# JADGardner/neusky

Hardware: AMD Instinct MI355X
Metric: train rays/sec on NeRF-OSR lk2 @1024 rays x 96 samples (higher is better)
Workload: dtype f32 in memory; forward products: fp16 hi + residual split, 3 x v_mfma_f32_32x32x16_f16 per product on power-of-two pre-scaled operands, one fp32 accumulator (~2^-22): FiLM-SIREN chains and the SDF / albedo field alike; backward products: the same fp16 split on per-row / per-matrix pre-scaled gradien; 1 GPU; full NeuSky train step (BASELINE configs[2]): 1024 rays/GPU x 96 samples, proposal 256+96, 512 illumination directions (256 upper-hemisphere DDF queries/ray), illumination decoder = this project's FiLM-SIREN H = 128 (RENI-shaped: latent 100x3; the reference's configured Attention decoder is absent from its tree), hash L16 F2 T2^19 x2, 256-wide MLPs; fwd + losses + bwd + all-reduce + 5 Adam groups; rays_per_gpu=1024, samples_per_ray=96, illumination_directions=512, parallelism=ray-sharded dp1, launcher=self-spawned, launch=HIP graph replay (1 graph/step + all-reduce + 5 Adam launches)

## Files before the change

neusky_amd/csrc/wgrad_native.hip:

```cpp
#include "common.h"
#include "../../include/neusky_hip.h"

namespace {

typedef _Float16 f16x8 __attribute__((ext_vector_type(8)));
typedef float f32x16 __attribute__((ext_vector_type(16)));
typedef float f32x4 __attribute__((ext_vector_type(4)));
typedef short s16x4 __attribute__((__vector_size__(4 * sizeof(short))));
typedef __attribute__((address_space(3))) s16x4 lds_s16x4;

struct WgradProblem {
  const float* A;
  const float* B;
  float* dW;
  float* db;
  const float* a_scale_max;
  float b_scale;
  const float* b_scale_max;
  int nnt_a, nnt_b, ldw;
  int tile0;
  int lda, ldb;
  int wa, wb;
  int bias_rows;
  int bias_mod;
};
struct WgradArgs {
  WgradProblem p[NSKY_WGRAD_MAX_PROBLEMS];
  int n_problems, rows, row_blocks, blocks_per_split, n_tiles;
};

__device__ __forceinline__ float pow2_scale(float m, float& inv) {
  if (!(m > 0.0f) || !(m < 3.0e38f)) { inv = 1.0f; return 1.0f; }
  int e;
  (void)frexpf(m, &e);
  e = max(-100, min(100, e));
  inv = ldexpf(1.0f, e - 15);
  return ldexpf(1.0f, 15 - e);
}

__device__ __forceinline__ int xcd_contiguous(int id, int total) {
  const int xcd = id & 7, idx = id >> 3, per = total >> 3, rem = total & 7;
  return xcd * per + min(xcd, rem) + idx;
}

template <bool BF>
__device__ __forceinline__ f32x16 mma(f16x8 x, f16x8 y, f32x16 acc) {
  typedef __bf16 b16x8 __attribute__((ext_vector_type(8)));
  if (BF) return __builtin_amdgcn_mfma_f32_32x32x16_bf16(__builtin_bit_cast(b16x8, x), __builtin_bit_cast(b16x8, y), acc, 0, 0, 0);
  return __builtin_amdgcn_mfma_f32_32x32x16_f16(x, y, acc, 0, 0, 0);
}

template <int WM, int WN, int TM, int TN, bool RM>
__global__ __launch_bounds__(64 * WM * WN, WM * WN == 8 ? 1 : 2) void wgrad_native_kernel(WgradArgs a) {
  constexpr int NW = WM * WN;
  constexpr int NT = NW;
  static_assert(WM * TM == NT && WN * TN == NT, "square output block");
  constexpr int OPB = NT * 4096;
  constexpr int STAGE = 2 * OPB;
  extern __shared__ __attribute__((aligned(16))) unsigned char smem[];

  const int tid = threadIdx.x, lane = tid & 63, wave = tid >> 6;
  const int wm = wave / WN, wn = wave % WN;
  const int logical = xcd_contiguous(blockIdx.x, gridDim.x);
  const int gtile = logical % a.n_tiles, split = logical / a.n_tiles;
  int pi = 0;
  while (pi + 1 < a.n_problems && gtile >= a.p[pi + 1].tile0) ++pi;
  const WgradProblem& P = a.p[pi];
  const int tile = gtile - P.tile0;
  const int kblocks = P.nnt_b / NT;
  const int nb = tile / kblocks, kb = tile % kblocks;
  const int r_beg = split * a.blocks_per_split;
  const int r_end = min(a.row_blocks, r_beg + a.blocks_per_split);
  if (r_beg >= r_end) return;

  float a_inv = 1.0f;
  const float a_scale = P.a_scale_max ? pow2_scale(*P.a_scale_max, a_inv) : 1.0f;
  float b_unused;
  const float b_scale = P.b_scale_max ? pow2_scale(*P.b_scale_max, b_unused) : P.b_scale;
  const bool clamp_b = P.b_scale_max == nullptr;

  const int c = lane & 31, hh = lane >> 5;
  const int rq = lane >> 3, fq = lane & 7;
  const int fa = (nb * NT + wave) * 32 + 4 * fq, fb = (kb * NT + wave) * 32 + 4 * fq;
  const bool fa_ok = fa < P.wa, fb_ok = fb < P.wb;
  const float* pa = RM ? P.A + (long)r_beg * 32 * P.lda + min(fa, max(P.wa - 4, 0))
                       : P.A + ((long)r_beg * P.nnt_a + nb * NT + wave) * 1024 + lane * 4;
  const float* pb = RM ? P.B + (long)r_beg * 32 * P.ldb + min(fb, max(P.wb - 4, 0))
                       : P.B + ((long)r_beg * P.nnt_b + kb * NT + wave) * 1024 + lane * 4;
  const long a_step = RM ? 32l * P.lda : (long)P.nnt_a * 1024, b_step = RM ? 32l * P.ldb : (long)P.nnt_b * 1024;
  int rm_row0 = 0;
  f32x4 raw[8];
  const float* pa2 = pa;
  const float* pb2 = pb;
  auto reload = [&](int uu) {
    if (RM) {
      const int row = min(rm_row0 + 8 * (uu >> 1) + rq, a.rows - 1) - rm_row0;
      raw[uu] = __builtin_nontemporal_load(reinterpret_cast<const f32x4*>(((uu & 1) ? pb2 + (long)row * P.ldb : pa2 + (long)row * P.lda)));
    } else {
      raw[uu] = __builtin_nontemporal_load(reinterpret_cast<const f32x4*>(((uu & 1) ? pb2 : pa2) + (uu >> 1) * 256));
    }
  };
  float bias[4][4];
#pragma unroll
  for (int u = 0; u < 4; ++u)
#pragma unroll
    for (int i = 0; i < 4; ++i) bias[u][i] = 0.0f;
  const bool want_bias = P.db != nullptr && kb == 0;
  const int w_base = wave * 4096 + c * 64 + 8 * hh;
  const int w_swz = (c >> 1) & 3;
  typedef _Float16 f16x4 __attribute__((ext_vector_type(4)));
  typedef __bf16 b16x4 __attribute__((ext_vector_type(4)));
  auto stage_unit = [&](int uu, int row0, bool row_block_live, unsigned char* stage) {
    const int op = uu & 1, u = uu >> 1;
    const float s = op == 0 ? a_scale : b_scale;
    const int row = row0 + (RM ? 8 * u + rq : c);
    const bool live = row_block_live && row < a.rows && (!RM || (op == 0 ? fa_ok : fb_ok));
    const bool bias_on = op == 0 && row < P.bias_rows && (P.bias_mod <= 1 || (row % P.bias_mod) == 0);
    float v[4];
#pragma unroll
    for (int i = 0; i < 4; ++i) {
      v[i] = live ? raw[uu][i] * s : 0.0f;
      if (op == 1 && clamp_b) v[i] = __builtin_amdgcn_fmed3f(v[i], -65504.0f, 65504.0f);
      if (op == 0) bias[u][i] += bias_on ? v[i] : 0.0f;
    }
    unsigned char* img;
    if (RM) {
      const int r = 8 * u + rq;
      img = stage + op * OPB + wave * 4096 + r * 64 + 16 * ((fq >> 1) ^ ((r >> 1) & 3)) + 8 * (fq & 1);
      b16x4 h4, l4;
#pragma unroll
      for (int i = 0; i < 4; ++i) { h4[i] = (__bf16)v[i]; l4[i] = (__bf16)(v[i] - (float)h4[i]); }
      *reinterpret_cast<b16x4*>(img) = h4;
      *reinterpret_cast<b16x4*>(img + 2048) = l4;
    } else {
      img = stage + op * OPB + w_base + 16 * (u ^ w_swz);
      f16x4 h4, l4;
#pragma unroll
      for (int i = 0; i < 4; ++i) { h4[i] = (_Float16)v[i]; l4[i] = (_Float16)(v[i] - (float)h4[i]); }
      *reinterpret_cast<f16x4*>(img) = h4;
      *reinterpret_cast<f16x4*>(img + 2048) = l4;
    }
  };

  const int i16 = lane & 15, q = i16 >> 2, p = i16 & 3, gsel = (lane >> 4) & 1, h = lane >> 5;
  int t_off[2];
#pragma unroll
  for (int rd = 0; rd < 2; ++rd) {
    const int row = 8 * h + 4 * rd + q;
    t_off[rd] = row * 64 + 16 * ((2 * gsel + (p >> 1)) ^ ((row >> 1) & 3)) + 8 * (p & 1);
  }
  auto frag = [&](const unsigned char* img, int ks) -> f16x8 {
    const s16x4 lo4 = __builtin_amdgcn_ds_read_tr16_b64_v4i16((lds_s16x4*)(img + ks * 1024 + t_off[0]));
    const s16x4 hi4 = __builtin_amdgcn_ds_read_tr16_b64_v4i16((lds_s16x4*)(img + ks * 1024 + t_off[1]));
    typedef short s16x8 __attribute__((ext_vector_type(8)));
    const s16x8 v = {lo4[0], lo4[1], lo4[2], lo4[3], hi4[0], hi4[1], hi4[2], hi4[3]};
    return __builtin_bit_cast(f16x8, v);
  };

  f32x16 acc[TM][TN];
#pragma unroll
  for (int i = 0; i < TM; ++i)
#pragma unroll
    for (int j = 0; j < TN; ++j)
#pragma unroll
      for (int r = 0; r < 16; ++r) acc[i][j][r] = 0.0f;

  rm_row0 = r_beg * 32;
#pragma unroll
  for (int uu = 0; uu < 8; ++uu) reload(uu);
  {
    if (r_beg + 1 < r_end) { pa2 += a_step; pb2 += b_step; rm_row0 += 32; }
#pragma unroll
    for (int uu = 0; uu < 8; ++uu) {
      stage_unit(uu, r_beg * 32, true, smem);
      reload(uu);
    }
    if (r_beg + 2 < r_end) { pa2 += a_step; pb2 += b_step; rm_row0 += 32; }
  }
  static_assert(TN == 4 || TN == 2, "one staging unit per (k-step, X tile) point, or two");
  constexpr int UPP = 8 / (2 * TN);
  int cur = 0;
  for (int r = r_beg; r < r_end; ++r) {
    __syncthreads();
    const bool live = r + 1 < r_end;
    const unsigned char* st = smem + cur * STAGE;
    unsigned char* nxt = smem + (cur ^ 1) * STAGE;
#pragma unroll
    for (int ks = 0; ks < 2; ++ks) {
      f16x8 ah[TM], al[TM], bh[2], bl[2];
#pragma unroll
      for (int i = 0; i < TM; ++i) {
        ah[i] = frag(st + (wm * TM + i) * 4096, ks);
        al[i] = frag(st + (wm * TM + i) * 4096 + 2048, ks);
      }
      bh[0] = frag(st + OPB + (wn * TN) * 4096, ks);
      bl[0] = frag(st + OPB + (wn * TN) * 4096 + 2048, ks);
#pragma unroll
      for (int j = 0; j < TN; ++j) {
        if (j + 1 < TN) {
          bh[(j + 1) & 1] = frag(st + OPB + (wn * TN + j + 1) * 4096, ks);
          bl[(j + 1) & 1] = frag(st + OPB + (wn * TN + j + 1) * 4096 + 2048, ks);
        }
#pragma unroll
        for (int i = 0; i < TM; ++i) acc[i][j] = mma<RM>(al[i], bh[j & 1], acc[i][j]);
#pragma unroll
        for (int i = 0; i < TM; ++i) acc[i][j] = mma<RM>(ah[i], bl[j & 1], acc[i][j]);
#pragma unroll
        for (int i = 0; i < TM; ++i) acc[i][j] = mma<RM>(ah[i], bh[j & 1], acc[i][j]);
#pragma unroll
        for (int k = 0; k < UPP; ++k) {
          const int uu = (ks * TN + j) * UPP + k;
          stage_unit(uu, (r + 1) * 32, live, nxt);
          reload(uu);
        }
        __builtin_amdgcn_sched_barrier(0);
      }
    }
    if (r + 3 < r_end) { pa2 += a_step; pb2 += b_step; rm_row0 += 32; }
    cur ^= 1;
  }

  const float out_scale = a_inv / b_scale;
  const int n0 = (nb * NT + wm * TM) * 32, k0 = (kb * NT + wn * TN) * 32;
#pragma unroll
  for (int i = 0; i < TM; ++i)
#pragma unroll
    for (int j = 0; j < TN; ++j) {
      float* out = P.dW + (long)(n0 + 32 * i + 4 * h) * P.ldw + k0 + 32 * j + (lane & 31);
      const bool col_ok = k0 + 32 * j + (lane & 31) < P.wb;
#pragma unroll
      for (int g = 0; g < 16; ++g)
        if (col_ok && n0 + 32 * i + 4 * h + 8 * (g >> 2) + (g & 3) < P.wa)
          atomicAdd(out + (long)(8 * (g >> 2) + (g & 3)) * P.ldw, acc[i][j][g] * out_scale);
      __builtin_amdgcn_sched_barrier(0);
    }
  if (want_bias && RM) {
#pragma unroll
    for (int i = 0; i < 4; ++i) {
      float v = (bias[0][i] + bias[1][i]) + (bias[2][i] + bias[3][i]);
#pragma unroll
      for (int off = 8; off < 64; off <<= 1) v += __shfl_xor(v, off, 64);
      if (rq == 0 && fa + i < P.wa) atomicAdd(P.db + fa + i, v * a_inv);
    }
  } else if (want_bias) {
#pragma unroll
    for (int u = 0; u < 4; ++u)
#pragma unroll
      for (int i = 0; i < 4; ++i) {
        float v = bias[u][i];
#pragma unroll
        for (int off = 16; off > 0; off >>= 1) v += __shfl_xor(v, off, 64);
        if (c == 0 && (nb * NT + wave) * 32 + 8 * u + 4 * hh + i < P.wa) atomicAdd(P.db + (nb * NT + wave) * 32 + 8 * u + 4 * hh + i, v * a_inv);
      }
  }
}

}

extern "C" int nsky_wgrad_native_batch(const nsky_wgrad_problem* problems, int32_t n_problems, int32_t rows, nsky_stream_t stream) {
  NSKY_CHECK_ARG(problems && n_problems >= 1 && n_problems <= NSKY_WGRAD_MAX_PROBLEMS && rows >= 0,
                 "nsky_wgrad_native_batch: 1..%d problems expected, got %d", NSKY_WGRAD_MAX_PROBLEMS, n_problems);
  if (rows == 0) return NSKY_OK;
  WgradArgs a;
  const bool rm = problems[0].lda > 0;
  bool wide = true;
  for (int i = 0; i < n_problems; ++i) {
    const nsky_wgrad_problem& q = problems[i];
    NSKY_CHECK_ARG(q.dZ && q.X && q.dW, "nsky_wgrad_native_batch: problem %d: null argument", i);
    NSKY_CHECK_ARG((q.lda > 0) == rm && (q.ldb > 0) == rm, "nsky_wgrad_native_batch: problem %d: row-major and tile-native operands in one launch", i);
    if (rm) {
      NSKY_CHECK_ARG(q.width_a >= 4 && q.width_b >= 4 && q.width_a % 4 == 0 && q.width_b % 4 == 0 && q.lda >= q.width_a && q.ldb >= q.width_b &&
                         q.lda % 4 == 0 && q.ldb % 4 == 0, "nsky_wgrad_native_batch: problem %d: row-major widths / leading dimensions must be multiples of 4", i);
      NSKY_CHECK_ARG(q.ldw >= q.width_b && q.a_scale_max == nullptr, "nsky_wgrad_native_batch: problem %d: ldw %d < %d, or a scale with row-major operands", i,
                     q.ldw, q.width_b);
      wide = wide && q.width_a > 128 && q.width_b > 128;
    } else {
      NSKY_CHECK_ARG(q.nnt_a > 0 && q.nnt_b > 0 && q.nnt_a % 4 == 0 && q.nnt_b % 4 == 0,
                     "nsky_wgrad_native_batch: problem %d: both operands need a multiple of 128 features (got %d and %d tiles of 32)", i,
                     q.nnt_a, q.nnt_b);
      NSKY_CHECK_ARG(q.width_a >= 0 && q.width_a <= 32 * q.nnt_a && q.width_b >= 0 && q.width_b <= 32 * q.nnt_b,
                     "nsky_wgrad_native_batch: problem %d: widths %d / %d exceed the tiles", i, q.width_a, q.width_b);
      NSKY_CHECK_ARG(q.ldw >= (q.width_b > 0 ? q.width_b : 32 * q.nnt_b), "nsky_wgrad_native_batch: problem %d: ldw %d too small", i, q.ldw);
      int e = 0;
      NSKY_CHECK_ARG(q.b_scale > 0.0f && frexpf(q.b_scale, &e) == 0.5f, "nsky_wgrad_native_batch: problem %d: b_scale must be a power of two", i);
      wide = wide && q.nnt_a % 8 == 0 && q.nnt_b % 8 == 0;
    }
  }
  const int NT = wide ? 8 : 4;
  int tiles = 0;
  for (int i = 0; i < n_problems; ++i) {
    const nsky_wgrad_problem& q = problems[i];
    WgradProblem& P = a.p[i];
    P.A = q.dZ; P.B = q.X; P.dW = q.dW; P.db = q.db; P.a_scale_max = q.a_scale_max; P.b_scale = rm ? 1.0f : q.b_scale;
    P.b_scale_max = rm ? nullptr : q.b_scale_max;
    P.nnt_a = rm ? ceil_div(q.width_a, 32 * NT) * NT : q.nnt_a;
    P.nnt_b = rm ? ceil_div(q.width_b, 32 * NT) * NT : q.nnt_b;
    P.ldw = q.ldw; P.tile0 = tiles;
    P.lda = q.lda; P.ldb = q.ldb;
    P.wa = (rm || q.width_a > 0) ? q.width_a : 32 * q.nnt_a;
    P.wb = (rm || q.width_b > 0) ? q.width_b : 32 * q.nnt_b;
    P.bias_rows = q.bias_rows > 0 ? q.bias_rows : rows;
    P.bias_mod = rm ? 0 : q.bias_row_mod;
    tiles += (P.nnt_a / NT) * (P.nnt_b / NT);
  }
  a.n_problems = n_problems; a.rows = rows; a.n_tiles = tiles;
  a.row_blocks = ceil_div(rows, 32);
  const int slots = wide ? 256 : 512;
  int splits = slots / a.n_tiles;
  if (splits < 1) splits = 1;
  if (splits > a.row_blocks) splits = a.row_blocks;
  a.blocks_per_split = ceil_div(a.row_blocks, splits);
  splits = ceil_div(a.row_blocks, a.blocks_per_split);
  const dim3 grid(a.n_tiles * splits);
  const size_t smem = 2 * 2 * NT * 4096;
  static bool attr_set = [] {
    (void)hipFuncSetAttribute(reinterpret_cast<const void*>(&wgrad_native_kernel<4, 2, 2, 4, false>), hipFuncAttributeMaxDynamicSharedMemorySize, 160 * 1024);
    (void)hipFuncSetAttribute(reinterpret_cast<const void*>(&wgrad_native_kernel<2, 2, 2, 2, false>), hipFuncAttributeMaxDynamicSharedMemorySize, 160 * 1024);
    (void)hipFuncSetAttribute(reinterpret_cast<const void*>(&wgrad_native_kernel<4, 2, 2, 4, true>), hipFuncAttributeMaxDynamicSharedMemorySize, 160 * 1024);
    (void)hipFuncSetAttribute(reinterpret_cast<const void*>(&wgrad_native_kernel<2, 2, 2, 2, true>), hipFuncAttributeMaxDynamicSharedMemorySize, 160 * 1024);
    return true;
  }();
  (void)attr_set;
  const hipStream_t st = (hipStream_t)stream;
  if (wide && rm) hipLaunchKernelGGL((wgrad_native_kernel<4, 2, 2, 4, true>), grid, dim3(512), smem, st, a);
  else if (wide) hipLaunchKernelGGL((wgrad_native_kernel<4, 2, 2, 4, false>), grid, dim3(512), smem, st, a);
  else if (rm) hipLaunchKernelGGL((wgrad_native_kernel<2, 2, 2, 2, true>), grid, dim3(256), smem, st, a);
  else hipLaunchKernelGGL((wgrad_native_kernel<2, 2, 2, 2, false>), grid, dim3(256), smem, st, a);
  NSKY_CHECK_LAUNCH("nsky_wgrad_native_batch");
  return NSKY_OK;
}

extern "C" int nsky_wgrad_native(const float* dZ, int32_t nnt_a, const float* X, int32_t nnt_b, int32_t rows, float* dW, int32_t ldw,
                                 float* db, const float* a_scale_max, float b_scale, nsky_stream_t stream) {
  nsky_wgrad_problem q = {};
  q.dZ = dZ; q.nnt_a = nnt_a; q.X = X; q.nnt_b = nnt_b; q.dW = dW; q.ldw = ldw; q.db = db; q.a_scale_max = a_scale_max; q.b_scale = b_scale;
  return nsky_wgrad_native_batch(&q, 1, rows, stream);
}
```

Before: 51650 rays/s.

## Software-pipeline LDS fragment reads across k-steps in weight-gradient kernel

Restructures the wgrad MFMA main loop so the A/B fragments for the next k-step (including the first k-step of the next row block) are read from LDS while the current MFMAs run, with a barrier per k-step in place of one per row block. It also remaps per-lane global load offsets to 32-bit byte offsets from a wave-uniform base, makes the wave index scalar, shrinks the bias accumulators and replaces the modulo bias-row test with a power-of-two mask and an FMA. The aim is to hide LDS latency and cut address and VGPR cost, in exchange for an extra barrier per k-step and more intricate staging/swizzle indexing.

```diff
diff --git a/neusky_amd/csrc/wgrad_native.hip b/neusky_amd/csrc/wgrad_native.hip
--- a/neusky_amd/csrc/wgrad_native.hip
+++ b/neusky_amd/csrc/wgrad_native.hip
@@ -23,6 +23,7 @@
   int wa, wb;
   int bias_rows;
   int bias_mod;
+  int bias_mask;
 };
 struct WgradArgs {
   WgradProblem p[NSKY_WGRAD_MAX_PROBLEMS];
@@ -59,7 +60,7 @@
   constexpr int STAGE = 2 * OPB;
   extern __shared__ __attribute__((aligned(16))) unsigned char smem[];
 
-  const int tid = threadIdx.x, lane = tid & 63, wave = tid >> 6;
+  const int tid = threadIdx.x, lane = tid & 63, wave = __builtin_amdgcn_readfirstlane(tid >> 6);
   const int wm = wave / WN, wn = wave % WN;
   const int logical = xcd_contiguous(blockIdx.x, gridDim.x);
   const int gtile = logical % a.n_tiles, split = logical / a.n_tiles;
@@ -79,30 +80,31 @@
   const float b_scale = P.b_scale_max ? pow2_scale(*P.b_scale_max, b_unused) : P.b_scale;
   const bool clamp_b = P.b_scale_max == nullptr;
 
-  const int c = lane & 31, hh = lane >> 5;
+  const int c = lane & 15, hh = (lane >> 4) & 1, us = lane >> 5;
   const int rq = lane >> 3, fq = lane & 7;
   const int fa = (nb * NT + wave) * 32 + 4 * fq, fb = (kb * NT + wave) * 32 + 4 * fq;
   const bool fa_ok = fa < P.wa, fb_ok = fb < P.wb;
-  const float* pa = RM ? P.A + (long)r_beg * 32 * P.lda + min(fa, max(P.wa - 4, 0))
-                       : P.A + ((long)r_beg * P.nnt_a + nb * NT + wave) * 1024 + lane * 4;
-  const float* pb = RM ? P.B + (long)r_beg * 32 * P.ldb + min(fb, max(P.wb - 4, 0))
-                       : P.B + ((long)r_beg * P.nnt_b + kb * NT + wave) * 1024 + lane * 4;
+  const float* pa2 = RM ? P.A + (long)r_beg * 32 * P.lda : P.A + ((long)r_beg * P.nnt_a + nb * NT + wave) * 1024;
+  const float* pb2 = RM ? P.B + (long)r_beg * 32 * P.ldb : P.B + ((long)r_beg * P.nnt_b + kb * NT + wave) * 1024;
   const long a_step = RM ? 32l * P.lda : (long)P.nnt_a * 1024, b_step = RM ? 32l * P.ldb : (long)P.nnt_b * 1024;
+  const unsigned lane_off = 4u * (us * 256 + hh * 128 + c * 4);
+  const unsigned fa_off = 4u * min(fa, max(P.wa - 4, 0)), fb_off = 4u * min(fb, max(P.wb - 4, 0));
   int rm_row0 = 0;
   f32x4 raw[8];
-  const float* pa2 = pa;
-  const float* pb2 = pb;
   auto reload = [&](int uu) {
+    const char* base = reinterpret_cast<const char*>((uu & 1) ? pb2 : pa2);
+    unsigned off;
     if (RM) {
-      const int row = min(rm_row0 + 8 * (uu >> 1) + rq, a.rows - 1) - rm_row0;
-      raw[uu] = __builtin_nontemporal_load(reinterpret_cast<const f32x4*>(((uu & 1) ? pb2 + (long)row * P.ldb : pa2 + (long)row * P.lda)));
+      const unsigned row = min(rm_row0 + 8 * (uu >> 1) + rq, a.rows - 1) - rm_row0;
+      off = (uu & 1) ? row * 4u * P.ldb + fb_off : row * 4u * P.lda + fa_off;
     } else {
-      raw[uu] = __builtin_nontemporal_load(reinterpret_cast<const f32x4*>(((uu & 1) ? pb2 : pa2) + (uu >> 1) * 256));
-    }
+      off = lane_off + 4u * (((uu >> 1) & 1) * 512 + (uu >> 2) * 64);
+    }
+    raw[uu] = __builtin_nontemporal_load(reinterpret_cast<const f32x4*>(base + off));
   };
-  float bias[4][4];
-#pragma unroll
-  for (int u = 0; u < 4; ++u)
+  float bias[2][4];
+#pragma unroll
+  for (int u = 0; u < 2; ++u)
 #pragma unroll
     for (int i = 0; i < 4; ++i) bias[u][i] = 0.0f;
   const bool want_bias = P.db != nullptr && kb == 0;
@@ -113,15 +115,18 @@
   auto stage_unit = [&](int uu, int row0, bool row_block_live, unsigned char* stage) {
     const int op = uu & 1, u = uu >> 1;
     const float s = op == 0 ? a_scale : b_scale;
-    const int row = row0 + (RM ? 8 * u + rq : c);
+    const int row = row0 + (RM ? 8 * u + rq : 16 * (u >> 1) + c);
     const bool live = row_block_live && row < a.rows && (!RM || (op == 0 ? fa_ok : fb_ok));
-    const bool bias_on = op == 0 && row < P.bias_rows && (P.bias_mod <= 1 || (row % P.bias_mod) == 0);
+    bool row_in = P.bias_mask >= 0 ? (row & P.bias_mask) == 0 : true;
+    if (P.bias_mask < 0 && P.bias_mod > 1) row_in = (row % P.bias_mod) == 0;
+    const bool bias_on = op == 0 && (row < P.bias_rows) & row_in;
+    const float bias_w = bias_on ? 1.0f : 0.0f;
     float v[4];
 #pragma unroll
     for (int i = 0; i < 4; ++i) {
       v[i] = live ? raw[uu][i] * s : 0.0f;
       if (op == 1 && clamp_b) v[i] = __builtin_amdgcn_fmed3f(v[i], -65504.0f, 65504.0f);
-      if (op == 0) bias[u][i] += bias_on ? v[i] : 0.0f;
+      if (op == 0) bias[RM ? 0 : u & 1][i] = __builtin_fmaf(v[i], bias_w, bias[RM ? 0 : u & 1][i]);
     }
     unsigned char* img;
     if (RM) {
@@ -133,7 +138,7 @@
       *reinterpret_cast<b16x4*>(img) = h4;
       *reinterpret_cast<b16x4*>(img + 2048) = l4;
     } else {
-      img = stage + op * OPB + w_base + 16 * (u ^ w_swz);
+      img = stage + op * OPB + w_base + (u >> 1) * 1024 + 16 * ((2 * (u & 1) + us) ^ w_swz);
       f16x4 h4, l4;
 #pragma unroll
       for (int i = 0; i < 4; ++i) { h4[i] = (_Float16)v[i]; l4[i] = (_Float16)(v[i] - (float)h4[i]); }
@@ -177,29 +182,39 @@
     }
     if (r_beg + 2 < r_end) { pa2 += a_step; pb2 += b_step; rm_row0 += 32; }
   }
-  static_assert(TN == 4 || TN == 2, "one staging unit per (k-step, X tile) point, or two");
-  constexpr int UPP = 8 / (2 * TN);
+  static_assert(TN == 4 || TN == 2, "one staging unit per X tile and slot, or two");
+  constexpr int UPP = 4 / TN;
+  __syncthreads();
+  f16x8 ah[TM], al[TM], bh[2], bl[2];
+#pragma unroll
+  for (int i = 0; i < TM; ++i) {
+    ah[i] = frag(smem + (wm * TM + i) * 4096, 0);
+    al[i] = frag(smem + (wm * TM + i) * 4096 + 2048, 0);
+  }
+  bh[0] = frag(smem + OPB + (wn * TN) * 4096, 0);
+  bl[0] = frag(smem + OPB + (wn * TN) * 4096 + 2048, 0);
   int cur = 0;
   for (int r = r_beg; r < r_end; ++r) {
-    __syncthreads();
     const bool live = r + 1 < r_end;
     const unsigned char* st = smem + cur * STAGE;
     unsigned char* nxt = smem + (cur ^ 1) * STAGE;
 #pragma unroll
     for (int ks = 0; ks < 2; ++ks) {
-      f16x8 ah[TM], al[TM], bh[2], bl[2];
-#pragma unroll
-      for (int i = 0; i < TM; ++i) {
-        ah[i] = frag(st + (wm * TM + i) * 4096, ks);
-        al[i] = frag(st + (wm * TM + i) * 4096 + 2048, ks);
-      }
-      bh[0] = frag(st + OPB + (wn * TN) * 4096, ks);
-      bl[0] = frag(st + OPB + (wn * TN) * 4096 + 2048, ks);
+      const unsigned char* sn = ks == 0 ? st : nxt;
+      const int kn = ks ^ 1;
+      f16x8 nh[TM], nl[TM];
 #pragma unroll
       for (int j = 0; j < TN; ++j) {
-        if (j + 1 < TN) {
-          bh[(j + 1) & 1] = frag(st + OPB + (wn * TN + j + 1) * 4096, ks);
-          bl[(j + 1) & 1] = frag(st + OPB + (wn * TN + j + 1) * 4096 + 2048, ks);
+        const unsigned char* bn = j + 1 < TN ? st + OPB + (wn * TN + j + 1) * 4096 : sn + OPB + (wn * TN) * 4096;
+        const int kb_ = j + 1 < TN ? ks : kn;
+        bh[(j + 1) & 1] = frag(bn, kb_);
+        bl[(j + 1) & 1] = frag(bn + 2048, kb_);
+        if (j == 0) {
+#pragma unroll
+          for (int i = 0; i < TM; ++i) {
+            nh[i] = frag(sn + (wm * TM + i) * 4096, kn);
+            nl[i] = frag(sn + (wm * TM + i) * 4096 + 2048, kn);
+          }
         }
 #pragma unroll
         for (int i = 0; i < TM; ++i) acc[i][j] = mma<RM>(al[i], bh[j & 1], acc[i][j]);
@@ -209,12 +224,15 @@
         for (int i = 0; i < TM; ++i) acc[i][j] = mma<RM>(ah[i], bh[j & 1], acc[i][j]);
 #pragma unroll
         for (int k = 0; k < UPP; ++k) {
-          const int uu = (ks * TN + j) * UPP + k;
+          const int uu = ks * 4 + j * UPP + k;
           stage_unit(uu, (r + 1) * 32, live, nxt);
           reload(uu);
         }
         __builtin_amdgcn_sched_barrier(0);
       }
+      __syncthreads();
+#pragma unroll
+      for (int i = 0; i < TM; ++i) { ah[i] = nh[i]; al[i] = nl[i]; }
     }
     if (r + 3 < r_end) { pa2 += a_step; pb2 += b_step; rm_row0 += 32; }
     cur ^= 1;
@@ -237,20 +255,21 @@
   if (want_bias && RM) {
 #pragma unroll
     for (int i = 0; i < 4; ++i) {
-      float v = (bias[0][i] + bias[1][i]) + (bias[2][i] + bias[3][i]);
+      float v = bias[0][i];
 #pragma unroll
       for (int off = 8; off < 64; off <<= 1) v += __shfl_xor(v, off, 64);
       if (rq == 0 && fa + i < P.wa) atomicAdd(P.db + fa + i, v * a_inv);
     }
   } else if (want_bias) {
 #pragma unroll
-    for (int u = 0; u < 4; ++u)
+    for (int u = 0; u < 2; ++u)
 #pragma unroll
       for (int i = 0; i < 4; ++i) {
         float v = bias[u][i];
 #pragma unroll
-        for (int off = 16; off > 0; off >>= 1) v += __shfl_xor(v, off, 64);
-        if (c == 0 && (nb * NT + wave) * 32 + 8 * u + 4 * hh + i < P.wa) atomicAdd(P.db + (nb * NT + wave) * 32 + 8 * u + 4 * hh + i, v * a_inv);
+        for (int off = 8; off > 0; off >>= 1) v += __shfl_xor(v, off, 64);
+        const int f = (nb * NT + wave) * 32 + 8 * (2 * u + us) + 4 * hh + i;
+        if (c == 0 && f < P.wa) atomicAdd(P.db + f, v * a_inv);
       }
   }
 }
@@ -301,6 +320,7 @@
     P.wb = (rm || q.width_b > 0) ? q.width_b : 32 * q.nnt_b;
     P.bias_rows = q.bias_rows > 0 ? q.bias_rows : rows;
     P.bias_mod = rm ? 0 : q.bias_row_mod;
+    P.bias_mask = (P.bias_mod > 1 && (P.bias_mod & (P.bias_mod - 1)) == 0) ? P.bias_mod - 1 : -1;
     tiles += (P.nnt_a / NT) * (P.nnt_b / NT);
   }
   a.n_problems = n_problems; a.rows = rows; a.n_tiles = tiles;
@@ -312,7 +332,7 @@
   a.blocks_per_split = ceil_div(a.row_blocks, splits);
   splits = ceil_div(a.row_blocks, a.blocks_per_split);
   const dim3 grid(a.n_tiles * splits);
-  const size_t smem = 2 * 2 * NT * 4096;
+  const size_t smem = 4 * 2 * NT * 2048;
   static bool attr_set = [] {
     (void)hipFuncSetAttribute(reinterpret_cast<const void*>(&wgrad_native_kernel<4, 2, 2, 4, false>), hipFuncAttributeMaxDynamicSharedMemorySize, 160 * 1024);
     (void)hipFuncSetAttribute(reinterpret_cast<const void*>(&wgrad_native_kernel<2, 2, 2, 2, false>), hipFuncAttributeMaxDynamicSharedMemorySize, 160 * 1024);
```

Result: no change. 51730 rays/s (median of 6 runs) (+0.2%).
